# EloDoyard/movie-recommender-system

Measured on AMD Instinct MI355X. Metric: test-set predictions/sec (kNN k=300, fit+predict+MAE), higher is better.
Workload: dtype fp16 MFMA similarity filter (fp32 acc) + f64 exact re-rank/prediction

## Files before the change

### movie-recommender-system_amd/csrc/api.cpp

```cpp
#include <math.h>
#include <stdio.h>
#include <string.h>

#include <algorithm>
#include <vector>

#include "engine.h"

using namespace knncf;

namespace knncf {
void launch_first_rows(int64_t n, const int32_t* d_du, const int32_t* d_di, int32_t own_lo, int32_t own_hi,
                       uint32_t* d_first, hipStream_t st);
void launch_length_keys(int32_t count, const int32_t* d_list, const int64_t* d_u_ptr, int32_t max_len, uint64_t* d_key, hipStream_t st);
void launch_collect_new(int32_t U, const uint32_t* d_first, int64_t* d_seq, int64_t epoch, int32_t own_lo, int32_t own_hi,
                        int32_t* d_list, int32_t* d_count, hipStream_t st);
void launch_fallback_keys(int32_t U, const double* d_exact, uint64_t* d_keys, uint32_t* d_vals, hipStream_t st);
void launch_fallback_write(int32_t user, int32_t take, int32_t kcap, const uint32_t* d_sorted_vals,
                           const double* d_exact, int32_t* nbr_idx, double* nbr_sim, int32_t* nbr_cnt,
                           hipStream_t st);
void launch_jaccard_pair(const Train& tr, int32_t u, int32_t v, double* d_out, hipStream_t st);
}

struct StageTimer {
    hipEvent_t a, b;
    double* acc;
};

struct knncf_handle {
    knncf_config cfg{};
    hipStream_t stream = nullptr;
    std::string err;
    Train tr;
    PrepScratch prep;
    bool fitted = false, committed = false;
    int8_t short_rows = -1;
    NeighborTable nt;
    int64_t epoch = 1;
    int64_t U_pad = 0, K_pad = 0;
    DArr<bf16_t> Bpanel;
    bool b_ready = false;
    int32_t head = 0;
    double tail_pairs_full = 0.0;
    DArr<int32_t> colmap;
    DArr<int32_t> te_cnt, te_item;
    DArr<float> te_x, row_tail_abs, row_head_sq;
    DArr<float> row_len;
    hipStream_t stream2 = nullptr;
    DArr<bf16_t> Apanel[2];
    DArr<float> S[2];
    DArr<float> S_full;
    DArr<uint32_t> sym_tiles;
    DArr<int32_t> redo_rows;
    int32_t sym_tiles_n = 0;
    hipEvent_t ev_produced[2] = {nullptr, nullptr}, ev_consumed[2] = {nullptr, nullptr}, ev_ready = nullptr;
    int32_t* pinned_cnt = nullptr;
    size_t pinned_cap = 0;
    SelectScratch sel;
    SliceScratch slices;
    NeighborTable pt;
    bool pt_ready = false;
    PersonalRows prow;
    bool prow_ready = false;
    DArr<int32_t> reco_users, reco_items, reco_out_items;
    DArr<double> reco_pred, reco_out_preds;
    DArr<uint8_t> reco_rated;
    QueryBatchScratch query_batch;
    RecoBatchScratch reco_batch;
    DArr<int32_t> build_list, build_count;
    DArr<uint32_t> first_row;
    DArr<int32_t> t_du, t_di, t_users, t_items;
    DArr<double> t_pred, t_err, t_ratings, t_partial, scalar_out;
    DArr<unsigned long long> scalar_u64;
    DArr<uint8_t> t_owned;
    DArr<int64_t> t_counts;
    DArr<int32_t> sweep_ks;
    std::vector<uint32_t> h_ukeys, h_ikeys;
    std::vector<int32_t> h_uid;
    knncf_timings tm{};
    std::vector<StageTimer> pending;
    std::vector<hipEvent_t> event_pool;
};

namespace {

hipEvent_t get_event(knncf_handle* h) {
    if (!h->event_pool.empty()) {
        hipEvent_t e = h->event_pool.back();
        h->event_pool.pop_back();
        return e;
    }
    hipEvent_t e;
    KN_HIP(hipEventCreate(&e));
    return e;
}

struct Stage {
    knncf_handle* h;
    StageTimer t;
    hipStream_t st;
    Stage(knncf_handle* h_, double* acc, hipStream_t st_ = nullptr) : h(h_), st(st_ ? st_ : h_->stream) {
        t.a = get_event(h);
        t.b = get_event(h);
        t.acc = acc;
        (void)hipEventRecord(t.a, st);
    }
    ~Stage() {
        (void)hipEventRecord(t.b, st);
        h->pending.push_back(t);
// ... 7 lines not shown
        float ms = 0.f;
        if (hipEventElapsedTime(&ms, t.a, t.b) == hipSuccess) *t.acc += ms;
        h->event_pool.push_back(t.a);
        h->event_pool.push_back(t.b);
    }
    h->pending.clear();
}

template <class F>
int guarded(knncf_handle* h, F&& f) {
    if (!h) return KNNCF_E_INVALID;
    struct DeviceGuard {
        int prev = -1;
        ~DeviceGuard() { if (prev >= 0) (void)hipSetDevice(prev); }
    } guard;
    try {
        int cur = -1;
        if (hipGetDevice(&cur) != hipSuccess) {
            (void)hipGetLastError();
            KN_HIP(hipSetDevice(h->cfg.device));
        } else if (cur != h->cfg.device) {
            guard.prev = cur;
            KN_HIP(hipSetDevice(h->cfg.device));
        }
        f();
        resolve_timers(h);
        return KNNCF_OK;
    } catch (const Error& e) {
        h->err = e.what();
        (void)hipStreamSynchronize(h->stream);
        (void)hipStreamSynchronize(h->stream2);
        (void)hipGetLastError();
        h->pending.clear();
        return e.status;
    } catch (const std::bad_alloc&) {
        h->err = "host allocation failed";
        return KNNCF_E_NOMEM;
    } catch (const std::exception& e) {
        h->err = e.what();
        return KNNCF_E_INVALID;
    }
}

void require_fitted(knncf_handle* h, bool committed = true) {
    KN_REQUIRE(h->fitted, KNNCF_E_STATE, "call knncf_fit first");
    if (committed) KN_REQUIRE(h->committed, KNNCF_E_STATE, "sharded handle: call knncf_shard_commit after the exchange");
}

void load_host_ids(knncf_handle* h) {
    if (!h->h_ukeys.empty() || h->tr.U == 0) return;
    Train& tr = h->tr;
    h->h_ukeys.resize(tr.U);
    h->h_ikeys.resize(tr.I);
    h->h_uid.resize(tr.U);
    KN_HIP(hipMemcpyAsync(h->h_ukeys.data(), tr.ukeys.p, tr.U * sizeof(uint32_t), hipMemcpyDeviceToHost, h->stream));
    KN_HIP(hipMemcpyAsync(h->h_ikeys.data(), tr.ikeys.p, tr.I * sizeof(uint32_t), hipMemcpyDeviceToHost, h->stream));
    KN_HIP(hipMemcpyAsync(h->h_uid.data(), tr.uid.p, tr.U * sizeof(int32_t), hipMemcpyDeviceToHost, h->stream));
    KN_HIP(hipStreamSynchronize(h->stream));
}

int32_t dense_user(knncf_handle* h, int32_t raw) {
    load_host_ids(h);
    return dense_lookup(h->h_ukeys.data(), h->tr.U, raw);
}
int32_t dense_item(knncf_handle* h, int32_t raw) {
    load_host_ids(h);
// ... 83 lines not shown
        }
        if (tr.jaccard && (h->cfg.flags & KNNCF_FLAG_F32_PANEL) == 0) H = std::min(H, 2048);
    }
    h->tail_pairs_full = tail_sq[H];
    return H;
}

void build_neighbors(knncf_handle* h, int32_t count) {
    Train& tr = h->tr;
    NeighborTable& nt = h->nt;
    if (count <= 0 || nt.kcap <= 0) return;
    KN_REQUIRE(h->cfg.similarity != KNNCF_SIM_ONE, KNNCF_E_UNSUPPORTED,
               "kNN neighbourhoods with similarityOne: every similarity is 1.0, the neighbourhood is the first k users in Set order — not built");
    hipStream_t st = h->stream;
    if (count > 256) {
        PrepScratch& sc = h->prep;
        sc.k64_a.ensure(count); sc.k64_b.ensure(count); sc.v32_b.ensure(count);
        launch_length_keys(count, h->build_list.p, tr.u_ptr.p, tr.I, sc.k64_a.p, st);
        sort_pairs_u64_u32(sc.sort, sc.k64_a.p, sc.k64_b.p, reinterpret_cast<const uint32_t*>(h->build_list.p), sc.v32_b.p, count, bits_for((uint64_t)tr.I), st);
        KN_HIP(hipMemcpyAsync(h->build_list.p, sc.v32_b.p, (size_t)count * sizeof(int32_t), hipMemcpyDeviceToDevice, st));
    }
    const bool fp16 = (h->cfg.flags & KNNCF_FLAG_BF16_FILTER) == 0;
    const bool s_fp16 = (h->cfg.flags & KNNCF_FLAG_F32_PANEL) == 0;
    h->U_pad = round_up(tr.U, 256);
    const int64_t U_pad = h->U_pad;
    size_t free_b = 0, total_b = 0;
    KN_HIP(hipMemGetInfo(&free_b, &total_b));
    const int64_t s_elem = s_fp16 ? 2 : 4;
    const size_t sym_bytes = (size_t)U_pad * (size_t)U_pad * (size_t)s_elem;
    size_t own = h->S_full.bytes() + h->sel.cand_idx.bytes() + h->sel.cand_approx.bytes() + h->sel.grp_v0.bytes() + h->sel.grp_x.bytes();
    for (int s = 0; s < 2; ++s) own += h->S[s].bytes() + h->Apanel[s].bytes();
    bool use_sym = h->cfg.shard_count == 1 && (int64_t)count * 2 >= tr.U && U_pad / 256 < 65536 &&
                   sym_bytes <= (free_b + own) / 3 && !getenv("KNNCF_DEBUG_NO_SYMMETRIC_GEMM");
    if (use_sym) {
        try {
            h->S_full.ensure((sym_bytes + 3) / 4);
        } catch (const Error& e) {
            if (e.status != KNNCF_E_NOMEM) throw;
            (void)hipGetLastError();
            use_sym = false;
        }
    }
    if (!h->b_ready) {
        h->head = choose_head(h, count, use_sym);
        h->K_pad = round_up(h->head, 64);
        size_t need = (size_t)U_pad * h->K_pad * sizeof(bf16_t);
        KN_REQUIRE(need < free_b + h->Bpanel.bytes(), KNNCF_E_UNSUPPORTED,
                   "dense bf16 user panel does not fit in HBM; lower head_items");
        Stage s(h, &h->tm.densify_ms);
        h->colmap.ensure(tr.I);
        launch_colmap(tr, h->head, h->colmap.p, st);
        h->Bpanel.ensure((size_t)U_pad * h->K_pad);
        launch_densify(tr, nullptr, 0, tr.U, h->colmap.p, h->Bpanel.p, h->K_pad, U_pad, fp16, st);
        if (tr.jaccard) {
            KN_REQUIRE(!s_fp16 || h->head <= 2048, KNNCF_E_UNSUPPORTED, "Jaccard: more than 2048 dense head items need KNNCF_FLAG_F32_PANEL");
            h->row_len.ensure((size_t)row_len_size(tr.U));
            launch_row_len(tr, h->row_len.p, st);
        }
        if (h->head < tr.I) {
            h->te_cnt.ensure(tr.U); h->te_item.ensure(tr.n); h->te_x.ensure(tr.n);
            h->row_tail_abs.ensure(tr.U); h->row_head_sq.ensure(tr.U);
            launch_tail_entries(tr, h->colmap.p, h->te_cnt.p, h->te_item.p, h->te_x.p, h->row_tail_abs.p, h->row_head_sq.p, st);
        }
        h->b_ready = true;
        KN_HIP(hipMemGetInfo(&free_b, &total_b));
    }
    const int64_t K_pad = h->K_pad;
    const int32_t head = h->head;
    h->tm.head_items = head;
    if (use_sym) {
        const int32_t n_tiles = (int32_t)(U_pad / 256);
        if (h->sym_tiles_n != n_tiles) {
            std::vector<uint32_t> list;
            gemm_sym_tile_list(n_tiles, list);
            h->sym_tiles.ensure(list.size());
            KN_HIP(hipMemcpyAsync(h->sym_tiles.p, list.data(), list.size() * sizeof(uint32_t), hipMemcpyHostToDevice, st));
            KN_HIP(hipStreamSynchronize(st));
            h->sym_tiles_n = n_tiles;
        }
        const int64_t n_listed = (int64_t)n_tiles * (n_tiles + 1) / 2;
        Stage s(h, &h->tm.gemm_ms);
        launch_gemm_sym(h->Bpanel.p, h->S_full.p, s_fp16, U_pad, h->K_pad, h->K_pad, U_pad, fp16, !tr.jaccard, h->sym_tiles.p, n_listed, st);
        h->tm.gemm_launches += 1;
        h->tm.gemm_flops_executed += 2.0 * 256.0 * 256.0 * (double)n_listed * (double)h->K_pad;
        h->tm.gemm_flops_algorithmic += 2.0 * (double)count * (double)(tr.U - 1) * (double)h->head;
        KN_HIP(hipMemGetInfo(&free_b, &total_b));
    } else {
        h->S_full.release();
    }
    size_t held = 0;
    for (int s = 0; s < 2; ++s) held += h->S[s].bytes() + h->Apanel[s].bytes();
    held += h->sel.cand_idx.bytes() + h->sel.cand_approx.bytes() + h->sel.grp_v0.bytes() + h->sel.grp_x.bytes();
    int64_t budget = h->cfg.workspace_bytes > 0 ? h->cfg.workspace_bytes / 2
                                                : (int64_t)std::min<size_t>((size_t)48 << 30, (free_b + held) / 4);
    int64_t per_row = (use_sym ? 0 : U_pad * s_elem + K_pad * 2) + (int64_t)shortlist_cap(nt.k, tr.U) * 8 + (int64_t)select_gcap(nt.k) * 36;
    if (h->cfg.workspace_bytes <= 0) {
        const int64_t whole = round_up(count, 256) * per_row;
        if (whole <= (int64_t)std::min<size_t>((size_t)96 << 30, (free_b + held) / 3)) budget = std::max(budget, whole);
    }
    int64_t R = std::max<int64_t>(256, (budget / per_row) / 256 * 256);
    R = std::min<int64_t>(R, round_up(count, 256));
    const int64_t n_blocks = ceil_div(count, R);
    R = round_up(ceil_div(count, n_blocks), 256);
    const bool overlap = (h->cfg.flags & KNNCF_FLAG_OVERLAP) != 0;
    const int slots = (overlap && n_blocks > 1 && !use_sym) ? 2 : 1;
    for (int s = 0; s < slots && !use_sym; ++s) {
        h->S[s].ensure((size_t)(R * U_pad * s_elem + 3) / 4);
        h->Apanel[s].ensure((size_t)R * K_pad);
    }
    const int32_t cap = shortlist_cap(nt.k, tr.U);
    const bool verify = (h->cfg.flags & KNNCF_FLAG_VERIFY_BOUND) != 0;
    h->sel.cand_idx.ensure((size_t)R * cap);
    h->sel.cand_approx.ensure((size_t)R * cap);
    h->sel.cand_cnt.ensure(R);
    h->sel.cand_eps.ensure(R);
    h->sel.row_entries.ensure(R);
    h->sel.grp_v0.ensure((size_t)R * select_gcap(nt.k));
    h->sel.grp_x.ensure((size_t)R * select_gcap(nt.k) * 8);
    h->sel.stats.ensure(4);
    KN_HIP(hipMemsetAsync(h->sel.stats.p, 0, 4 * sizeof(double), st));
    if (h->pinned_cap < (size_t)count) {
        if (h->pinned_cnt) KN_HIP(hipHostFree(h->pinned_cnt));
        h->pinned_cnt = nullptr;
        h->pinned_cap = 0;
        KN_HIP(hipHostMalloc((void**)&h->pinned_cnt, (size_t)count * sizeof(int32_t), hipHostMallocDefault));
        h->pinned_cap = (size_t)count;
    }
    const float eps_opnd = gemm_eps_operand(fp16);
    const float eps_rest = gemm_eps_rest(fp16) + (s_fp16 ? 2.45e-4f : 0.f);
    hipStream_t sp = slots > 1 ? h->stream2 : h->stream;
    hipStream_t sc = h->stream;
    KN_HIP(hipEventRecord(h->ev_ready, sc));
    KN_HIP(hipStreamWaitEvent(sp, h->ev_ready, 0));
    std::vector<int32_t> h_rows;
    auto need_h_rows = [&] {
        if (!h_rows.empty()) return;
        h_rows.resize(count);
        KN_HIP(hipMemcpyAsync(h_rows.data(), h->build_list.p, (size_t)count * sizeof(int32_t), hipMemcpyDeviceToHost, st));
        KN_HIP(hipStreamSynchronize(st));
    };
    auto redo_marked = [&](const std::vector<int32_t>& marked, const void* Sp, bool by_user, int64_t rb) {
        need_h_rows();
        std::vector<int32_t> users(marked.size()), srow(marked.size());
        for (size_t j = 0; j < marked.size(); ++j) {
            users[j] = h_rows[marked[j]];
            srow[j] = (int32_t)(marked[j] - rb);
        }
        TailEntries te{h->te_cnt.p, h->te_item.p, h->te_x.p, h->row_tail_abs.p, h->row_head_sq.p, h->row_len.p};
        const int64_t chunk = std::min<int64_t>((int64_t)marked.size(), R);
        h->redo_rows.ensure(2 * (size_t)chunk);
        for (size_t j0 = 0; j0 < marked.size(); j0 += (size_t)R) {
            const int32_t m = (int32_t)std::min<size_t>((size_t)R, marked.size() - j0);
            KN_HIP(hipMemcpyAsync(h->redo_rows.p, users.data() + j0, (size_t)m * sizeof(int32_t), hipMemcpyHostToDevice, st));
            KN_HIP(hipMemcpyAsync(h->redo_rows.p + chunk, srow.data() + j0, (size_t)m * sizeof(int32_t), hipMemcpyHostToDevice, st));
            {
                Stage s(h, &h->tm.select_ms);
                launch_tail_select(tr, h->colmap.p, te, head < tr.I, Sp, by_user, s_fp16, U_pad, m, h->redo_rows.p, nt.k, eps_opnd, eps_rest, cap,
                                   h->sel.cand_idx.p, h->sel.cand_approx.p, h->sel.cand_cnt.p, h->sel.cand_eps.p, h->sel.grp_v0.p, h->sel.grp_x.p,
                                   select_gcap(nt.k), st, false, by_user ? nullptr : h->redo_rows.p + chunk);
                h->tm.select_launches += 1;
            }
            {
                Stage s(h, &h->tm.rerank_ms);
                launch_rerank(tr, nt, m, h->redo_rows.p, cap, h->sel.cand_idx.p, h->sel.cand_approx.p, h->sel.cand_cnt.p, h->sel.cand_eps.p,
                              h->sel.stats.p, h->sel.row_entries.p, verify, st);
            }
            std::vector<int32_t> again(m);
            KN_HIP(hipMemcpyAsync(again.data(), h->sel.cand_cnt.p, (size_t)m * sizeof(int32_t), hipMemcpyDeviceToHost, st));
            KN_HIP(hipStreamSynchronize(st));
            for (int32_t j = 0; j < m; ++j) h->pinned_cnt[marked[j0 + j]] = again[j];
        }
    };
    const bool per_block_redo = !use_sym && n_blocks > 1;
    for (int64_t b = 0; b < n_blocks; ++b) {
        const int64_t rb = b * R;
        const int32_t rows = (int32_t)std::min<int64_t>(R, count - rb);
        const int64_t M = round_up(rows, 256);
        const int32_t* d_rows = h->build_list.p + rb;
        const int slot = (int)(b % slots);
        if (b >= slots) KN_HIP(hipStreamWaitEvent(sp, h->ev_consumed[slot], 0));
        if (!use_sym) {
            Stage s(h, &h->tm.densify_ms, sp);
            launch_densify(tr, d_rows, 0, rows, h->colmap.p, h->Apanel[slot].p, K_pad, M, fp16, sp);
        }
        if (!use_sym) {
            Stage s(h, &h->tm.gemm_ms, sp);
            launch_gemm_nt(h->Apanel[slot].p, h->Bpanel.p, h->S[slot].p, s_fp16, M, U_pad, K_pad, K_pad, K_pad, U_pad, fp16, !tr.jaccard, sp);
            h->tm.gemm_launches += 1;
            h->tm.gemm_flops_executed += 2.0 * (double)M * (double)U_pad * (double)K_pad;
            h->tm.gemm_flops_algorithmic += 2.0 * (double)rows * (double)(tr.U - 1) * (double)head;
        }
        KN_HIP(hipEventRecord(h->ev_produced[slot], sp));
        KN_HIP(hipStreamWaitEvent(sc, h->ev_produced[slot], 0));
        TailEntries te{h->te_cnt.p, h->te_item.p, h->te_x.p, h->row_tail_abs.p, h->row_head_sq.p, h->row_len.p};
        h->prep.join_commit(sc);
        const void* Sblk = use_sym ? (const void*)h->S_full.p : (const void*)h->S[slot].p;
        const int32_t gcap = select_gcap(nt.k);
        auto select_rows = [&](int32_t r0, int32_t nr) {
            Stage s(h, &h->tm.select_ms, sc);
            const void* Sp = use_sym ? Sblk : (const void*)(static_cast<const char*>(Sblk) + (size_t)r0 * (size_t)U_pad * (size_t)s_elem);
            launch_tail_select(tr, h->colmap.p, te, head < tr.I, Sp, use_sym, s_fp16, U_pad, nr, d_rows + r0, nt.k, eps_opnd, eps_rest, cap,
                               h->sel.cand_idx.p + (size_t)r0 * cap, h->sel.cand_approx.p + (size_t)r0 * cap, h->sel.cand_cnt.p + r0, h->sel.cand_eps.p + r0,
                               h->sel.grp_v0.p + (size_t)r0 * gcap, h->sel.grp_x.p + (size_t)r0 * gcap * 8, gcap, sc);
            h->tm.select_launches += 1;
            h->tm.tail_pair_updates += h->tail_pairs_full * ((double)nr / (double)tr.U);
            h->tm.select_row_bytes += (double)s_elem * (double)nr * (double)tr.U;
        };
        const int32_t slices = std::min<int32_t>(8, 8192 / std::max<int32_t>(nt.kcap, 1));
        const char* force_slices = getenv("KNNCF_DEBUG_SLICE_ROWS");
        const int32_t n_heavy = slices < 2                         ? 0
                                : force_slices                     ? std::max<int32_t>(0, std::min<int32_t>(rows, atoi(force_slices)))
                                : (rows >= 4096 && rows <= 65536)  ? std::max<int32_t>(16, rows / 512)
                                                                   : 0;
        select_rows(0, rows);
        if (overlap && !per_block_redo) KN_HIP(hipEventRecord(h->ev_consumed[slot], sc));
        {
            Stage s(h, &h->tm.rerank_ms, sc);
            launch_rerank(tr, nt, rows, d_rows, cap, h->sel.cand_idx.p, h->sel.cand_approx.p, h->sel.cand_cnt.p, h->sel.cand_eps.p, h->sel.stats.p,
                          h->sel.row_entries.p, verify, sc, n_heavy, slices, &h->slices);
        }
        if (!overlap) KN_HIP(hipEventRecord(h->ev_consumed[slot], sc));
        if (per_block_redo) KN_HIP(hipMemcpyAsync(h->pinned_cnt + rb, h->sel.cand_cnt.p, rows * sizeof(int32_t), hipMemcpyDeviceToHost, sc));
        if (per_block_redo) {
            KN_HIP(hipStreamSynchronize(sc));
            std::vector<int32_t> marked;
            for (int64_t r = rb; r < rb + rows; ++r)
                if (h->pinned_cnt[r] > cap) marked.push_back((int32_t)r);
            if ((int64_t)marked.size() > std::max<int64_t>(64, rows / 200)) {
                redo_marked(marked, h->S[slot].p, false, rb);
            }
            if (overlap) KN_HIP(hipEventRecord(h->ev_consumed[slot], sc));
        }
    }
    const bool summary = !per_block_redo;
    unsigned long long four[4] = {0, 0, 0, 0};
    nt.by_id_valid = false;
    if (summary) KN_HIP(hipMemcpyAsync(four, h->sel.stats.p, sizeof(four), hipMemcpyDeviceToHost, sc));
    KN_HIP(hipStreamSynchronize(sc));
    KN_HIP(hipStreamSynchronize(sp));
    auto take_stats = [&](const unsigned long long* w) {
        h->tm.rerank_row_bytes += 12.0 * (double)w[1];
        if (verify && w[0] != 0) {
            double shifted;
            memcpy(&shifted, &w[0], sizeof(double));
            h->tm.max_bound_violation = std::max(h->tm.max_bound_violation, shifted - 4.0);
        }
// ... 15 lines not shown
    }
    for (int64_t r = 0; r < count; ++r) {
        h->tm.shortlist_total += std::min(h->pinned_cnt[r], cap);
        if (h->pinned_cnt[r] > cap) {
            need_h_rows();
            Stage s(h, &h->tm.rerank_ms);
            int32_t u = h_rows[r];
            h->sel.row_exact.ensure(tr.U);
            h->sel.fb_keys_a.ensure(tr.U); h->sel.fb_keys_b.ensure(tr.U);
            h->sel.fb_vals_a.ensure(tr.U); h->sel.fb_vals_b.ensure(tr.U);
            int64_t seq_u = fetch(h, nt.seq.p, u);
            launch_exact_row(tr, nt, u, seq_u, h->sel.row_exact.p, st);
            launch_fallback_keys(tr.U, h->sel.row_exact.p, h->sel.fb_keys_a.p, h->sel.fb_vals_a.p, st);
            sort_pairs_u64_u32(h->prep.sort, h->sel.fb_keys_a.p, h->sel.fb_keys_b.p, h->sel.fb_vals_a.p,
                               h->sel.fb_vals_b.p, tr.U, 64, st);
            launch_fallback_write(u, nt.kcap, nt.kcap, h->sel.fb_vals_b.p, h->sel.row_exact.p, nt.idx.p, nt.sim.p,
                                  nt.cnt.p, st);
            h->tm.fallback_rows += 1;
        }
    }
    {
        unsigned long long two[2] = {0, 0};
        KN_HIP(hipMemcpyAsync(two, h->sel.stats.p, sizeof(two), hipMemcpyDeviceToHost, st));
        KN_HIP(hipStreamSynchronize(st));
        take_stats(two);
    }
}

void ensure_test_scratch(knncf_handle* h, int64_t n) {
    h->t_du.ensure(n); h->t_di.ensure(n); h->t_pred.ensure(n); h->t_err.ensure(n); h->t_owned.ensure(n);
    h->t_partial.ensure(1024); h->t_counts.ensure(1024);
}

void ensure_neighbors_for_rows(knncf_handle* h, int64_t n) {
    Train& tr = h->tr;
    if (tr.U < 2 || h->nt.kcap <= 0) return;
    KN_REQUIRE(n < (int64_t)0xffffffffll, KNNCF_E_UNSUPPORTED, "more than 2^32-1 test rows");
    hipStream_t st = h->stream;
    h->first_row.ensure(tr.U);
    h->build_list.ensure(tr.U);
    h->build_count.ensure(1);
    KN_HIP(hipMemsetAsync(h->first_row.p, 0xff, tr.U * sizeof(uint32_t), st));
    KN_HIP(hipMemsetAsync(h->build_count.p, 0, sizeof(int32_t), st));
    launch_first_rows(n, h->t_du.p, h->t_di.p, 0, tr.U, h->first_row.p, st);
    launch_collect_new(tr.U, h->first_row.p, h->nt.seq.p, h->epoch, tr.own_lo, tr.own_hi, h->build_list.p, h->build_count.p, st);
    h->epoch += 1;
    int32_t count = fetch(h, h->build_count.p, 0);
    build_neighbors(h, count);
}

bool personalized_streams(const knncf_handle* h) { return h->tr.U > 2048 || getenv("KNNCF_DEBUG_PERSONALIZED_STREAM"); }

void require_personalized(knncf_handle* h) {
    Train& tr = h->tr;
    KN_REQUIRE(h->cfg.shard_count == 1, KNNCF_E_UNSUPPORTED, "PERSONALIZED is not sharded");
    if (h->cfg.similarity == KNNCF_SIM_COSINE) {
        std::vector<int64_t> ptr((size_t)tr.U + 1);
        KN_HIP(hipMemcpyAsync(ptr.data(), tr.u_ptr.p, ptr.size() * sizeof(int64_t), hipMemcpyDeviceToHost, h->stream));
        KN_HIP(hipStreamSynchronize(h->stream));
        for (int32_t u = 0; u < tr.U; ++u)
            KN_REQUIRE(ptr[u + 1] - ptr[u] > 4, KNNCF_E_UNSUPPORTED,
                       "PERSONALIZED with the adjusted cosine: a user with <= 4 ratings makes the reference's summation order depend on its memo history pair by pair (SURVEY N6); not modelled");
    }
}

void ensure_personalized_table(knncf_handle* h) {
    if (h->pt_ready) return;
    Train& tr = h->tr;
    require_personalized(h);
    NeighborTable& pt = h->pt;
    pt.k = pt.kcap = tr.U;
    const size_t cells = (size_t)tr.U * (size_t)tr.U;
    pt.uidx.ensure(cells);
    pt.usim.ensure(cells);
    pt.cnt.ensure(tr.U);
    launch_full_rows(tr, h->cfg.similarity == KNNCF_SIM_JACCARD, pt.uidx.p, pt.usim.p, pt.cnt.p, h->stream);
    pt.by_id_valid = true;
    h->pt_ready = true;
}

void ensure_personal_rows(knncf_handle* h) {
// ... 40 lines not shown
                                                          : (int64_t)std::min<size_t>((size_t)48 << 30, (free_b + pr.S.bytes()) / 4);
        R = std::min<int64_t>(std::max<int64_t>(1, budget / row_bytes), nu);
        R = ceil_div(nu, ceil_div(nu, R));
        pr.S.ensure((size_t)R * tr.U);
        std::vector<int32_t> slot((size_t)tr.U, -1);
        for (int64_t k = 0; k < nu; ++k) slot[users[k]] = (int32_t)(k % R);
        pr.users.ensure(nu);
        pr.slot.ensure(tr.U);
        KN_HIP(hipMemcpyAsync(pr.users.p, users.data(), (size_t)nu * sizeof(int32_t), hipMemcpyHostToDevice, st));
        KN_HIP(hipMemcpyAsync(pr.slot.p, slot.data(), (size_t)tr.U * sizeof(int32_t), hipMemcpyHostToDevice, st));
        KN_HIP(hipStreamSynchronize(st));
    }
    const int64_t n_blocks = std::max<int64_t>(1, ceil_div(nu, R));
    for (int64_t b = 0; b < n_blocks; ++b) {
        const int64_t u0 = b * R, u1 = std::min<int64_t>(nu, u0 + R);
        const int64_t r0 = b == 0 ? 0 : first_row[u0], r1 = b + 1 < n_blocks ? first_row[u1] : n;
        if (u1 > u0) {
            Stage s(h, &h->tm.rerank_ms);
            launch_sim_rows(tr, pr, pr.users.p + u0, (int32_t)(u1 - u0), pr.S.p, st);
        }
        Stage s(h, &h->tm.predict_ms);
        launch_fold_rows(tr, pr, r1 - r0, sc.v32_b.p + r0, h->t_du.p, h->t_di.p, d_ratings, pr.slot.p, pr.S.p, d_pred, h->t_err.p,
                         h->t_owned.p, st);
    }
}

void ensure_item_stats(knncf_handle* h) {
    if (h->tr.item_stats_ready) return;
    Stage s(h, &h->tm.prep_ms);
    h->prep.join_commit(h->stream);
    prep_item_stats(h->tr, h->prep, h->stream);
}

int64_t order_test_rows(knncf_handle* h, int64_t n, bool by_item, int32_t cols) {
    Train& tr = h->tr;
    hipStream_t st = h->stream;
    PrepScratch& sc = h->prep;
    sc.k64_a.ensure(n); sc.k64_b.ensure(n); sc.v32_a.ensure(n); sc.v32_b.ensure(n);
    const uint32_t key_limit = (uint32_t)(by_item ? tr.I : tr.U);
    if (h->cfg.shard_count > 1) {
        h->scalar_u64.ensure(1);
        KN_HIP(hipMemsetAsync(h->scalar_u64.p, 0, sizeof(unsigned long long), st));
        KN_HIP(hipMemsetAsync(h->t_err.p, 0, (size_t)cols * (size_t)n * sizeof(double), st));
        KN_HIP(hipMemsetAsync(h->t_owned.p, 0, (size_t)n, st));
        launch_owned_keys(n, by_item ? h->t_di.p : h->t_du.p, h->t_du.p, tr.own_lo, tr.own_hi, h->cfg.shard_rank == 0, key_limit,
                          sc.k64_a.p, sc.v32_a.p, h->scalar_u64.p, st);
        sort_pairs_u64_u32(sc.sort, sc.k64_a.p, sc.k64_b.p, sc.v32_a.p, sc.v32_b.p, n, bits_for((uint64_t)key_limit + 1), st);
        return (int64_t)fetch(h, h->scalar_u64.p, 0);
    }
    launch_user_keys(n, by_item ? h->t_di.p : h->t_du.p, key_limit, sc.k64_a.p, sc.v32_a.p, st);
    sort_pairs_u64_u32(sc.sort, sc.k64_a.p, sc.k64_b.p, sc.v32_a.p, sc.v32_b.p, n, bits_for((uint64_t)key_limit), st);
    return n;
}

void reduce_errors(knncf_handle* h, int64_t n, int32_t cols, double* sums, int64_t* count) {
    hipStream_t st = h->stream;
    const int32_t nb = 1024;
    h->t_partial.ensure((size_t)nb * cols);
    h->t_counts.ensure((size_t)nb * cols);
    for (int32_t c = 0; c < cols; ++c)
        launch_reduce_err(h->t_err.p + (size_t)c * n, h->t_owned.p, n, h->t_partial.p + (size_t)c * nb, h->t_counts.p + (size_t)c * nb, nb, st);
    std::vector<double> hp((size_t)nb * cols);
    std::vector<int64_t> hc((size_t)nb * cols);
    KN_HIP(hipMemcpyAsync(hp.data(), h->t_partial.p, hp.size() * sizeof(double), hipMemcpyDeviceToHost, st));
    KN_HIP(hipMemcpyAsync(hc.data(), h->t_counts.p, hc.size() * sizeof(int64_t), hipMemcpyDeviceToHost, st));
    KN_HIP(hipStreamSynchronize(st));
    for (int32_t c = 0; c < cols; ++c) {
        double s_ = 0.0;
        int64_t c_ = 0;
        for (int32_t b = 0; b < nb; ++b) { s_ += hp[(size_t)c * nb + b]; c_ += hc[(size_t)c * nb + b]; }
        if (sums) sums[c] = s_;
        if (count && c == 0) *count = c_;
    }
}

void run_predict(knncf_handle* h, int predictor, const int32_t* d_users, const int32_t* d_items,
                 const double* d_ratings, int64_t n, double* sum_abs_err, int64_t* count, double* d_pred_out) {
    require_fitted(h);
    Train& tr = h->tr;
    hipStream_t st = h->stream;
    KN_REQUIRE(n >= 0, KNNCF_E_INVALID, "negative row count");
    if (sum_abs_err) *sum_abs_err = 0.0;
    if (count) *count = 0;
    if (n == 0) return;
    KN_REQUIRE(d_users && d_items, KNNCF_E_INVALID, "null test arrays");
    int kind = predictor;
    NeighborTable* table = &h->nt;
    bool stream = false;
    if (predictor == KNNCF_PRED_PERSONALIZED) {
        if (h->cfg.similarity == KNNCF_SIM_ONE) {
            kind = KNNCF_PRED_BASELINE_RDD;
        } else if (personalized_streams(h)) {
            ensure_personal_rows(h);
            stream = true;
        } else {
            ensure_personalized_table(h);
            kind = KNNCF_PRED_KNN;
            table = &h->pt;
        }
    }
    KN_REQUIRE(stream || (kind >= KNNCF_PRED_GLOBAL_AVG && kind <= KNNCF_PRED_KNN), KNNCF_E_INVALID, "unknown predictor");
    if (kind == KNNCF_PRED_ITEM_AVG || kind == KNNCF_PRED_BASELINE || kind == KNNCF_PRED_BASELINE_RDD) ensure_item_stats(h);
    ensure_test_scratch(h, n);
    {
        Stage s(h, &h->tm.predict_ms);
        launch_dense_ids(tr, d_users, d_items, n, h->t_du.p, h->t_di.p, st);
    }
    if (kind == KNNCF_PRED_KNN && table == &h->nt) ensure_neighbors_for_rows(h, n);
    h->prep.join_commit(st);
    double* pred = d_pred_out ? d_pred_out : h->t_pred.p;
    if (stream) predict_personal_rows(h, d_ratings, n, pred);
    {
        Stage s(h, &h->tm.predict_ms);
        const uint32_t* d_order = nullptr;
        const bool by_item = tr.ib_words > 0 && lds_bitmap_fits(tr.ib_words);
        int64_t n_rows = n;
        if (kind == KNNCF_PRED_KNN) {
            n_rows = order_test_rows(h, n, by_item, 1);
            d_order = h->prep.v32_b.p;
        }
        if (n_rows > 0 && !stream)
            launch_predict(tr, table, kind, n_rows, h->t_du.p, h->t_di.p, d_ratings, d_order, by_item, pred, h->t_err.p, h->t_owned.p,
                           h->cfg.shard_rank == 0, st);
        if (sum_abs_err || count) reduce_errors(h, n, 1, sum_abs_err, count);
    }
}

void check_sweep_ks(const int32_t* ks, int32_t n_k) {
    KN_REQUIRE(ks && n_k >= 1 && n_k <= 64, KNNCF_E_INVALID, "sweep: 1 .. 64 values of k");
    for (int32_t q = 0; q < n_k; ++q)
        KN_REQUIRE(ks[q] >= 1 && ks[q] <= 2048 && (q == 0 || ks[q] > ks[q - 1]), KNNCF_E_INVALID,
                   "sweep: k must be strictly ascending in [1, 2048]");
}

void run_mae_sweep(knncf_handle* h, const int32_t* ks, int32_t n_k, const int32_t* d_users, const int32_t* d_items,
                   const double* d_ratings, int64_t n, double* sums, int64_t* count, double* d_pred) {
    check_sweep_ks(ks, n_k);
    require_fitted(h);
    KN_REQUIRE(h->cfg.similarity != KNNCF_SIM_ONE, KNNCF_E_UNSUPPORTED,
               "kNN neighbourhoods with similarityOne: every similarity is 1.0, the neighbourhood is the first k users in Set order — not built");
    KN_REQUIRE(n >= 0, KNNCF_E_INVALID, "negative row count");
    for (int32_t q = 0; q < n_k; ++q) sums[q] = 0.0;
    *count = 0;
    if (n == 0) return;
    KN_REQUIRE(d_users && d_items && d_ratings, KNNCF_E_INVALID, "null test arrays");
    Train& tr = h->tr;
    hipStream_t st = h->stream;
    struct Restore {
        knncf_handle* h;
        int32_t k;
        ~Restore() {
            h->cfg.k = k;
            try { reset_neighbors(h); } catch (const Error&) {}
        }
    } restore{h, h->cfg.k};
    h->cfg.k = ks[n_k - 1];
    reset_neighbors(h);
    ensure_test_scratch(h, n);
    h->t_err.ensure((size_t)n_k * n);
    {
        Stage s(h, &h->tm.predict_ms);
        launch_dense_ids(tr, d_users, d_items, n, h->t_du.p, h->t_di.p, st);
    }
    ensure_neighbors_for_rows(h, n);
    h->prep.join_commit(st);
    std::vector<int32_t> hk(ks, ks + n_k);
    h->sweep_ks.ensure(64);
    KN_HIP(hipMemcpyAsync(h->sweep_ks.p, hk.data(), (size_t)n_k * sizeof(int32_t), hipMemcpyHostToDevice, st));
    {
        Stage s(h, &h->tm.predict_ms);
        const int64_t n_rows = order_test_rows(h, n, true, n_k);
        if (n_rows > 0)
            launch_predict_sweep(tr, h->nt, h->sweep_ks.p, n_k, n_rows, n, h->t_du.p, h->t_di.p, d_ratings, h->prep.v32_b.p, d_pred,
                                 h->t_err.p, h->t_owned.p, h->cfg.shard_rank == 0, st);
        reduce_errors(h, n, n_k, sums, count);
    }
}

void do_fit_device(knncf_handle* h, const int32_t* d_users, const int32_t* d_items, const double* d_ratings, int64_t n) {
    KN_REQUIRE(n > 0 && d_users && d_items && d_ratings, KNNCF_E_INVALID, "fit: null or empty input");
    Train& tr = h->tr;
    hipStream_t st = h->stream;
    h->fitted = h->committed = false;
    h->short_rows = -1;
    h->b_ready = false;
    h->pt_ready = false;
    h->prow_ready = false;
    h->h_ukeys.clear(); h->h_ikeys.clear(); h->h_uid.clear();
    tr.n = n;
    tr.jaccard = h->cfg.similarity == KNNCF_SIM_JACCARD;
    {
        Stage s(h, &h->tm.prep_ms);
        if (tr.user_raw.p != d_users) {
            tr.user_raw.alloc(n); tr.item_raw.alloc(n); tr.rating.alloc(n);
            KN_HIP(hipMemcpyAsync(tr.user_raw.p, d_users, n * sizeof(int32_t), hipMemcpyDeviceToDevice, st));
            KN_HIP(hipMemcpyAsync(tr.item_raw.p, d_items, n * sizeof(int32_t), hipMemcpyDeviceToDevice, st));
            KN_HIP(hipMemcpyAsync(tr.rating.p, d_ratings, n * sizeof(double), hipMemcpyDeviceToDevice, st));
        }
        prep_fit(tr, h->prep, h->cfg.shard_rank, h->cfg.shard_count, st);
    }
    h->fitted = true;
    reset_neighbors(h);
    if (h->cfg.shard_count == 1) {
        Stage s(h, &h->tm.prep_ms);
        prep_commit(tr, h->prep, st);
        h->committed = true;
// ... 345 lines not shown
        case KNNCF_E_DUPLICATE: return "duplicate (user,item) rating";
        case KNNCF_E_NOMEM: return "out of memory";
        case KNNCF_E_HIP: return "HIP runtime error";
        case KNNCF_E_STATE: return "invalid call order";
        case KNNCF_E_UNSUPPORTED: return "unsupported configuration";
        case KNNCF_E_NODEVICE: return "no usable gfx950 device";
        case KNNCF_E_RCCL: return "RCCL error";
        default: return "unknown status";
    }
}

int knncf_create(const knncf_config* cfg, knncf_handle** out) {
    if (!cfg || !out || cfg->struct_size != sizeof(knncf_config)) return KNNCF_E_INVALID;
    if (cfg->shard_count < 1 || cfg->shard_rank < 0 || cfg->shard_rank >= cfg->shard_count || cfg->k < 0)
        return KNNCF_E_INVALID;
    if (cfg->similarity < KNNCF_SIM_COSINE || cfg->similarity > KNNCF_SIM_JACCARD) return KNNCF_E_INVALID;
    int ndev = 0;
    if (hipGetDeviceCount(&ndev) != hipSuccess || ndev <= 0 || cfg->device < 0 || cfg->device >= ndev) {
        (void)hipGetLastError();
        return KNNCF_E_NODEVICE;
    }
    hipDeviceProp_t prop;
    if (hipGetDeviceProperties(&prop, cfg->device) != hipSuccess) return KNNCF_E_NODEVICE;
    if (strncmp(prop.gcnArchName, "gfx950", 6) != 0) return KNNCF_E_NODEVICE;
    knncf_handle* h = new (std::nothrow) knncf_handle();
    if (!h) return KNNCF_E_NOMEM;
    h->cfg = *cfg;
    if (hipSetDevice(cfg->device) != hipSuccess || hipStreamCreateWithFlags(&h->stream, hipStreamNonBlocking) != hipSuccess ||
        hipStreamCreateWithFlags(&h->stream2, hipStreamNonBlocking) != hipSuccess) {
        delete h;
        return KNNCF_E_HIP;
    }
    bool ok = hipEventCreateWithFlags(&h->ev_ready, hipEventDisableTiming) == hipSuccess;
    for (int s = 0; s < 2; ++s) {
        ok = ok && hipEventCreateWithFlags(&h->ev_produced[s], hipEventDisableTiming) == hipSuccess;
        ok = ok && hipEventCreateWithFlags(&h->ev_consumed[s], hipEventDisableTiming) == hipSuccess;
    }
    if (!ok) {
        knncf_destroy(h);
        return KNNCF_E_HIP;
    }
    *out = h;
    return KNNCF_OK;
}

void knncf_destroy(knncf_handle* h) {
    if (!h) return;
    (void)hipSetDevice(h->cfg.device);
    (void)hipStreamSynchronize(h->stream);
    for (auto& t : h->pending) { (void)hipEventDestroy(t.a); (void)hipEventDestroy(t.b); }
    for (auto e : h->event_pool) (void)hipEventDestroy(e);
    if (h->stream2) (void)hipStreamSynchronize(h->stream2);
    if (h->ev_ready) (void)hipEventDestroy(h->ev_ready);
    for (int s = 0; s < 2; ++s) {
        if (h->ev_produced[s]) (void)hipEventDestroy(h->ev_produced[s]);
        if (h->ev_consumed[s]) (void)hipEventDestroy(h->ev_consumed[s]);
    }
    if (h->pinned_cnt) (void)hipHostFree(h->pinned_cnt);
    if (h->stream2) (void)hipStreamDestroy(h->stream2);
    (void)hipStreamDestroy(h->stream);
    delete h;
}

const char* knncf_last_error(const knncf_handle* h) { return h ? h->err.c_str() : "null handle"; }

int knncf_fit_device(knncf_handle* h, const int32_t* d_users, const int32_t* d_items, const double* d_ratings, int64_t n) {
    return guarded(h, [&] { do_fit_device(h, d_users, d_items, d_ratings, n); });
}

int knncf_fit(knncf_handle* h, const int32_t* users, const int32_t* items, const double* ratings, int64_t n) {
    return guarded(h, [&] {
        KN_REQUIRE(n > 0 && users && items && ratings, KNNCF_E_INVALID, "fit: null or empty input");
        Train& tr = h->tr;
        tr.user_raw.alloc(n); tr.item_raw.alloc(n); tr.rating.alloc(n);
        KN_HIP(hipMemcpyAsync(tr.user_raw.p, users, n * sizeof(int32_t), hipMemcpyHostToDevice, h->stream));
        KN_HIP(hipMemcpyAsync(tr.item_raw.p, items, n * sizeof(int32_t), hipMemcpyHostToDevice, h->stream));
        KN_HIP(hipMemcpyAsync(tr.rating.p, ratings, n * sizeof(double), hipMemcpyHostToDevice, h->stream));
        do_fit_device(h, tr.user_raw.p, tr.item_raw.p, tr.rating.p, n);
    });
}

int knncf_num_users(const knncf_handle* h, int32_t* out) {
    if (!h || !out || !h->fitted) return KNNCF_E_STATE;
    *out = h->tr.U;
    return KNNCF_OK;
}
// ... 535 lines not shown
```

Before: 85.76 million.

## Overlap tail-list build and test-row ordering with neighbor build on side stream

Tail-entry and row-length construction now run on the second stream after colmap, concurrently with densify and GEMM, and are joined only where the redo and select steps need them. Test-row key sorting moves to dedicated buffers and can run on the side stream beside the neighbor build. The post-build hipMemGetInfo calls are dropped in favour of bookkeeping over buffer sizes, and the symmetric tile list is uploaded earlier. This hides small kernels and host syncs behind the main build, at the cost of more events, extra scratch memory and cross-stream ordering that must stay correct.

After: 85.59 million. About the same (-0.2%).

```diff
diff --git a/movie-recommender-system_amd/csrc/api.cpp b/movie-recommender-system_amd/csrc/api.cpp
--- a/movie-recommender-system_amd/csrc/api.cpp
+++ b/movie-recommender-system_amd/csrc/api.cpp
@@ -54,6 +54,9 @@
     DArr<int32_t> redo_rows;
     int32_t sym_tiles_n = 0;
     hipEvent_t ev_produced[2] = {nullptr, nullptr}, ev_consumed[2] = {nullptr, nullptr}, ev_ready = nullptr;
+    hipEvent_t ev_colmap = nullptr, ev_tail = nullptr, ev_rows = nullptr;
+    bool tail_pending = false, rows_pending = false;
+    struct { bool want = false; int64_t n = 0; bool by_item = false; int32_t cols = 0; } rows_deferred;
     int32_t* pinned_cnt = nullptr;
     size_t pinned_cap = 0;
     SelectScratch sel;
@@ -75,6 +78,9 @@
     DArr<uint8_t> t_owned;
     DArr<int64_t> t_counts;
     DArr<int32_t> sweep_ks;
+    SortWorkspace t_sort;
+    DArr<uint64_t> t_k64_a, t_k64_b;
+    DArr<uint32_t> t_v32_a, t_order;
     std::vector<uint32_t> h_ukeys, h_ikeys;
     std::vector<int32_t> h_uid;
     knncf_timings tm{};
@@ -148,6 +154,7 @@
         (void)hipStreamSynchronize(h->stream2);
         (void)hipGetLastError();
         h->pending.clear();
+        h->tail_pending = h->rows_pending = h->rows_deferred.want = false;
         return e.status;
     } catch (const std::bad_alloc&) {
         h->err = "host allocation failed";
@@ -297,6 +304,7 @@
     for (int s = 0; s < 2; ++s) own += h->S[s].bytes() + h->Apanel[s].bytes();
     bool use_sym = h->cfg.shard_count == 1 && (int64_t)count * 2 >= tr.U && U_pad / 256 < 65536 &&
                    sym_bytes <= (free_b + own) / 3 && !getenv("KNNCF_DEBUG_NO_SYMMETRIC_GEMM");
+    const size_t s_full_before = h->S_full.bytes();
     if (use_sym) {
         try {
             h->S_full.ensure((sym_bytes + 3) / 4);
@@ -306,53 +314,86 @@
             use_sym = false;
         }
     }
+    auto build_bytes = [&] {
+        return h->S_full.bytes() + h->Bpanel.bytes() + h->colmap.bytes() + h->te_cnt.bytes() + h->te_item.bytes() + h->te_x.bytes() +
+               h->row_tail_abs.bytes() + h->row_head_sq.bytes() + h->row_len.bytes() + h->sym_tiles.bytes();
+    };
+    const size_t bytes_at_query = build_bytes() - h->S_full.bytes() + s_full_before;
+    const int32_t n_tiles = (int32_t)(U_pad / 256);
+    if (use_sym && h->sym_tiles_n != n_tiles) {
+        std::vector<uint32_t> list;
+        gemm_sym_tile_list(n_tiles, list);
+        h->sym_tiles.ensure(list.size());
+        KN_HIP(hipMemcpyAsync(h->sym_tiles.p, list.data(), list.size() * sizeof(uint32_t), hipMemcpyHostToDevice, st));
+        KN_HIP(hipStreamSynchronize(st));
+        h->sym_tiles_n = n_tiles;
+    }
+    const bool overlap = (h->cfg.flags & KNNCF_FLAG_OVERLAP) != 0;
+    auto launch_tail_lists = [&](hipStream_t side) {
+        {
+            Stage s(h, &h->tm.densify_ms, side);
+            if (tr.jaccard) launch_row_len(tr, h->row_len.p, side);
+            if (h->head < tr.I)
+                launch_tail_entries(tr, h->colmap.p, h->te_cnt.p, h->te_item.p, h->te_x.p, h->row_tail_abs.p, h->row_head_sq.p, side);
+        }
+        if (side != h->stream) {
+            KN_HIP(hipEventRecord(h->ev_tail, side));
+            h->tail_pending = true;
+        }
+    };
+    auto join_tail_lists = [&](hipStream_t consumer) {
+        if (!h->tail_pending) return;
+        KN_HIP(hipStreamWaitEvent(consumer, h->ev_tail, 0));
+        h->tail_pending = false;
+    };
+    bool tail_deferred = false;
     if (!h->b_ready) {
         h->head = choose_head(h, count, use_sym);
         h->K_pad = round_up(h->head, 64);
         size_t need = (size_t)U_pad * h->K_pad * sizeof(bf16_t);
         KN_REQUIRE(need < free_b + h->Bpanel.bytes(), KNNCF_E_UNSUPPORTED,
                    "dense bf16 user panel does not fit in HBM; lower head_items");
-        Stage s(h, &h->tm.densify_ms);
+        KN_REQUIRE(!tr.jaccard || !s_fp16 || h->head <= 2048, KNNCF_E_UNSUPPORTED, "Jaccard: more than 2048 dense head items need KNNCF_FLAG_F32_PANEL");
+        const bool has_tail = h->head < tr.I;
         h->colmap.ensure(tr.I);
-        launch_colmap(tr, h->head, h->colmap.p, st);
         h->Bpanel.ensure((size_t)U_pad * h->K_pad);
-        launch_densify(tr, nullptr, 0, tr.U, h->colmap.p, h->Bpanel.p, h->K_pad, U_pad, fp16, st);
-        if (tr.jaccard) {
-            KN_REQUIRE(!s_fp16 || h->head <= 2048, KNNCF_E_UNSUPPORTED, "Jaccard: more than 2048 dense head items need KNNCF_FLAG_F32_PANEL");
-            h->row_len.ensure((size_t)row_len_size(tr.U));
-            launch_row_len(tr, h->row_len.p, st);
-        }
-        if (h->head < tr.I) {
+        if (tr.jaccard) h->row_len.ensure((size_t)row_len_size(tr.U));
+        if (has_tail) {
             h->te_cnt.ensure(tr.U); h->te_item.ensure(tr.n); h->te_x.ensure(tr.n);
             h->row_tail_abs.ensure(tr.U); h->row_head_sq.ensure(tr.U);
-            launch_tail_entries(tr, h->colmap.p, h->te_cnt.p, h->te_item.p, h->te_x.p, h->row_tail_abs.p, h->row_head_sq.p, st);
+        }
+        {
+            Stage s(h, &h->tm.densify_ms);
+            launch_colmap(tr, h->head, h->colmap.p, st);
+            KN_HIP(hipEventRecord(h->ev_colmap, st));
+            launch_densify(tr, nullptr, 0, tr.U, h->colmap.p, h->Bpanel.p, h->K_pad, U_pad, fp16, st);
+        }
+        if (tr.jaccard || has_tail) {
+            if (overlap && !use_sym) {
+                tail_deferred = true;
+            } else {
+                KN_HIP(hipStreamWaitEvent(h->stream2, h->ev_colmap, 0));
+                launch_tail_lists(h->stream2);
+            }
         }
         h->b_ready = true;
-        KN_HIP(hipMemGetInfo(&free_b, &total_b));
     }
     const int64_t K_pad = h->K_pad;
     const int32_t head = h->head;
     h->tm.head_items = head;
     if (use_sym) {
-        const int32_t n_tiles = (int32_t)(U_pad / 256);
-        if (h->sym_tiles_n != n_tiles) {
-            std::vector<uint32_t> list;
-            gemm_sym_tile_list(n_tiles, list);
-            h->sym_tiles.ensure(list.size());
-            KN_HIP(hipMemcpyAsync(h->sym_tiles.p, list.data(), list.size() * sizeof(uint32_t), hipMemcpyHostToDevice, st));
-            KN_HIP(hipStreamSynchronize(st));
-            h->sym_tiles_n = n_tiles;
-        }
         const int64_t n_listed = (int64_t)n_tiles * (n_tiles + 1) / 2;
         Stage s(h, &h->tm.gemm_ms);
         launch_gemm_sym(h->Bpanel.p, h->S_full.p, s_fp16, U_pad, h->K_pad, h->K_pad, U_pad, fp16, !tr.jaccard, h->sym_tiles.p, n_listed, st);
         h->tm.gemm_launches += 1;
         h->tm.gemm_flops_executed += 2.0 * 256.0 * 256.0 * (double)n_listed * (double)h->K_pad;
         h->tm.gemm_flops_algorithmic += 2.0 * (double)count * (double)(tr.U - 1) * (double)h->head;
-        KN_HIP(hipMemGetInfo(&free_b, &total_b));
-    } else {
-        h->S_full.release();
-    }
+    }
+    {
+        const size_t now = build_bytes();
+        free_b = now >= bytes_at_query ? free_b - std::min(free_b, now - bytes_at_query) : free_b + (bytes_at_query - now);
+    }
+    if (!use_sym) h->S_full.release();
     size_t held = 0;
     for (int s = 0; s < 2; ++s) held += h->S[s].bytes() + h->Apanel[s].bytes();
     held += h->sel.cand_idx.bytes() + h->sel.cand_approx.bytes() + h->sel.grp_v0.bytes() + h->sel.grp_x.bytes();
@@ -367,7 +408,6 @@
     R = std::min<int64_t>(R, round_up(count, 256));
     const int64_t n_blocks = ceil_div(count, R);
     R = round_up(ceil_div(count, n_blocks), 256);
-    const bool overlap = (h->cfg.flags & KNNCF_FLAG_OVERLAP) != 0;
     const int slots = (overlap && n_blocks > 1 && !use_sym) ? 2 : 1;
     for (int s = 0; s < slots && !use_sym; ++s) {
         h->S[s].ensure((size_t)(R * U_pad * s_elem + 3) / 4);
@@ -397,6 +437,11 @@
     hipStream_t sc = h->stream;
     KN_HIP(hipEventRecord(h->ev_ready, sc));
     KN_HIP(hipStreamWaitEvent(sp, h->ev_ready, 0));
+    if (tail_deferred) {
+        hipStream_t side = slots > 1 ? sc : h->stream2;
+        if (side != sc) KN_HIP(hipStreamWaitEvent(side, h->ev_ready, 0));
+        launch_tail_lists(side);
+    }
     std::vector<int32_t> h_rows;
     auto need_h_rows = [&] {
         if (!h_rows.empty()) return;
@@ -412,6 +457,7 @@
             srow[j] = (int32_t)(marked[j] - rb);
         }
         TailEntries te{h->te_cnt.p, h->te_item.p, h->te_x.p, h->row_tail_abs.p, h->row_head_sq.p, h->row_len.p};
+        join_tail_lists(st);
         const int64_t chunk = std::min<int64_t>((int64_t)marked.size(), R);
         h->redo_rows.ensure(2 * (size_t)chunk);
         for (size_t j0 = 0; j0 < marked.size(); j0 += (size_t)R) {
@@ -477,6 +523,7 @@
                                 : force_slices                     ? std::max<int32_t>(0, std::min<int32_t>(rows, atoi(force_slices)))
                                 : (rows >= 4096 && rows <= 65536)  ? std::max<int32_t>(16, rows / 512)
                                                                    : 0;
+        join_tail_lists(sc);
         select_rows(0, rows);
         if (overlap && !per_block_redo) KN_HIP(hipEventRecord(h->ev_consumed[slot], sc));
         {
@@ -558,9 +605,9 @@
     h->t_partial.ensure(1024); h->t_counts.ensure(1024);
 }
 
-void ensure_neighbors_for_rows(knncf_handle* h, int64_t n) {
+int32_t collect_neighbors_for_rows(knncf_handle* h, int64_t n) {
     Train& tr = h->tr;
-    if (tr.U < 2 || h->nt.kcap <= 0) return;
+    if (tr.U < 2 || h->nt.kcap <= 0) return 0;
     KN_REQUIRE(n < (int64_t)0xffffffffll, KNNCF_E_UNSUPPORTED, "more than 2^32-1 test rows");
     hipStream_t st = h->stream;
     h->first_row.ensure(tr.U);
@@ -571,8 +618,7 @@
     launch_first_rows(n, h->t_du.p, h->t_di.p, 0, tr.U, h->first_row.p, st);
     launch_collect_new(tr.U, h->first_row.p, h->nt.seq.p, h->epoch, tr.own_lo, tr.own_hi, h->build_list.p, h->build_count.p, st);
     h->epoch += 1;
-    int32_t count = fetch(h, h->build_count.p, 0);
-    build_neighbors(h, count);
+    return fetch(h, h->build_count.p, 0);
 }
 
 bool personalized_streams(const knncf_handle* h) { return h->tr.U > 2048 || getenv("KNNCF_DEBUG_PERSONALIZED_STREAM"); }
@@ -679,25 +725,59 @@
     prep_item_stats(h->tr, h->prep, h->stream);
 }
 
-int64_t order_test_rows(knncf_handle* h, int64_t n, bool by_item, int32_t cols) {
+void order_test_rows(knncf_handle* h, int64_t n, bool by_item, int32_t cols, hipStream_t st) {
     Train& tr = h->tr;
-    hipStream_t st = h->stream;
-    PrepScratch& sc = h->prep;
-    sc.k64_a.ensure(n); sc.k64_b.ensure(n); sc.v32_a.ensure(n); sc.v32_b.ensure(n);
     const uint32_t key_limit = (uint32_t)(by_item ? tr.I : tr.U);
     if (h->cfg.shard_count > 1) {
-        h->scalar_u64.ensure(1);
         KN_HIP(hipMemsetAsync(h->scalar_u64.p, 0, sizeof(unsigned long long), st));
         KN_HIP(hipMemsetAsync(h->t_err.p, 0, (size_t)cols * (size_t)n * sizeof(double), st));
         KN_HIP(hipMemsetAsync(h->t_owned.p, 0, (size_t)n, st));
         launch_owned_keys(n, by_item ? h->t_di.p : h->t_du.p, h->t_du.p, tr.own_lo, tr.own_hi, h->cfg.shard_rank == 0, key_limit,
-                          sc.k64_a.p, sc.v32_a.p, h->scalar_u64.p, st);
-        sort_pairs_u64_u32(sc.sort, sc.k64_a.p, sc.k64_b.p, sc.v32_a.p, sc.v32_b.p, n, bits_for((uint64_t)key_limit + 1), st);
-        return (int64_t)fetch(h, h->scalar_u64.p, 0);
-    }
-    launch_user_keys(n, by_item ? h->t_di.p : h->t_du.p, key_limit, sc.k64_a.p, sc.v32_a.p, st);
-    sort_pairs_u64_u32(sc.sort, sc.k64_a.p, sc.k64_b.p, sc.v32_a.p, sc.v32_b.p, n, bits_for((uint64_t)key_limit), st);
-    return n;
+                          h->t_k64_a.p, h->t_v32_a.p, h->scalar_u64.p, st);
+        sort_pairs_u64_u32(h->t_sort, h->t_k64_a.p, h->t_k64_b.p, h->t_v32_a.p, h->t_order.p, n, bits_for((uint64_t)key_limit + 1), st);
+        return;
+    }
+    launch_user_keys(n, by_item ? h->t_di.p : h->t_du.p, key_limit, h->t_k64_a.p, h->t_v32_a.p, st);
+    sort_pairs_u64_u32(h->t_sort, h->t_k64_a.p, h->t_k64_b.p, h->t_v32_a.p, h->t_order.p, n, bits_for((uint64_t)key_limit), st);
+}
+int64_t ordered_row_count(knncf_handle* h, int64_t n) {
+    return h->cfg.shard_count > 1 ? (int64_t)fetch(h, h->scalar_u64.p, 0) : n;
+}
+
+void fork_test_order(knncf_handle* h);
+void queue_test_order(knncf_handle* h, int64_t n, bool by_item, int32_t cols, bool beside_build) {
+    h->t_k64_a.ensure(n); h->t_k64_b.ensure(n); h->t_v32_a.ensure(n); h->t_order.ensure(n);
+    if (h->cfg.shard_count > 1) h->scalar_u64.ensure(1);
+    if (beside_build && (h->cfg.flags & KNNCF_FLAG_OVERLAP) == 0) {
+        h->rows_deferred.want = true;
+        h->rows_deferred.n = n; h->rows_deferred.by_item = by_item; h->rows_deferred.cols = cols;
+        fork_test_order(h);
+        return;
+    }
+    Stage s(h, &h->tm.predict_ms);
+    order_test_rows(h, n, by_item, cols, h->stream);
+}
+void fork_test_order(knncf_handle* h) {
+    if (!h->rows_deferred.want) return;
+    h->rows_deferred.want = false;
+    KN_HIP(hipEventRecord(h->ev_rows, h->stream));
+    KN_HIP(hipStreamWaitEvent(h->stream2, h->ev_rows, 0));
+    {
+        Stage s(h, &h->tm.predict_ms, h->stream2);
+        order_test_rows(h, h->rows_deferred.n, h->rows_deferred.by_item, h->rows_deferred.cols, h->stream2);
+    }
+    KN_HIP(hipEventRecord(h->ev_rows, h->stream2));
+    h->rows_pending = true;
+}
+void join_test_order(knncf_handle* h) {
+    if (h->rows_deferred.want) {
+        h->rows_deferred.want = false;
+        Stage s(h, &h->tm.predict_ms);
+        order_test_rows(h, h->rows_deferred.n, h->rows_deferred.by_item, h->rows_deferred.cols, h->stream);
+    }
+    if (!h->rows_pending) return;
+    KN_HIP(hipStreamWaitEvent(h->stream, h->ev_rows, 0));
+    h->rows_pending = false;
 }
 
 void reduce_errors(knncf_handle* h, int64_t n, int32_t cols, double* sums, int64_t* count) {
@@ -753,18 +833,23 @@
         Stage s(h, &h->tm.predict_ms);
         launch_dense_ids(tr, d_users, d_items, n, h->t_du.p, h->t_di.p, st);
     }
-    if (kind == KNNCF_PRED_KNN && table == &h->nt) ensure_neighbors_for_rows(h, n);
+    const bool by_item = tr.ib_words > 0 && lds_bitmap_fits(tr.ib_words);
+    if (kind == KNNCF_PRED_KNN) {
+        const int32_t count = table == &h->nt ? collect_neighbors_for_rows(h, n) : 0;
+        queue_test_order(h, n, by_item, 1, count > 0);
+        build_neighbors(h, count);
+    }
     h->prep.join_commit(st);
     double* pred = d_pred_out ? d_pred_out : h->t_pred.p;
     if (stream) predict_personal_rows(h, d_ratings, n, pred);
     {
         Stage s(h, &h->tm.predict_ms);
         const uint32_t* d_order = nullptr;
-        const bool by_item = tr.ib_words > 0 && lds_bitmap_fits(tr.ib_words);
         int64_t n_rows = n;
         if (kind == KNNCF_PRED_KNN) {
-            n_rows = order_test_rows(h, n, by_item, 1);
-            d_order = h->prep.v32_b.p;
+            join_test_order(h);
+            n_rows = ordered_row_count(h, n);
+            d_order = h->t_order.p;
         }
         if (n_rows > 0 && !stream)
             launch_predict(tr, table, kind, n_rows, h->t_du.p, h->t_di.p, d_ratings, d_order, by_item, pred, h->t_err.p, h->t_owned.p,
@@ -809,16 +894,21 @@
         Stage s(h, &h->tm.predict_ms);
         launch_dense_ids(tr, d_users, d_items, n, h->t_du.p, h->t_di.p, st);
     }
-    ensure_neighbors_for_rows(h, n);
+    {
+        const int32_t count = collect_neighbors_for_rows(h, n);
+        queue_test_order(h, n, true, n_k, count > 0);
+        build_neighbors(h, count);
+    }
     h->prep.join_commit(st);
     std::vector<int32_t> hk(ks, ks + n_k);
     h->sweep_ks.ensure(64);
     KN_HIP(hipMemcpyAsync(h->sweep_ks.p, hk.data(), (size_t)n_k * sizeof(int32_t), hipMemcpyHostToDevice, st));
     {
         Stage s(h, &h->tm.predict_ms);
-        const int64_t n_rows = order_test_rows(h, n, true, n_k);
+        join_test_order(h);
+        const int64_t n_rows = ordered_row_count(h, n);
         if (n_rows > 0)
-            launch_predict_sweep(tr, h->nt, h->sweep_ks.p, n_k, n_rows, n, h->t_du.p, h->t_di.p, d_ratings, h->prep.v32_b.p, d_pred,
+            launch_predict_sweep(tr, h->nt, h->sweep_ks.p, n_k, n_rows, n, h->t_du.p, h->t_di.p, d_ratings, h->t_order.p, d_pred,
                                  h->t_err.p, h->t_owned.p, h->cfg.shard_rank == 0, st);
         reduce_errors(h, n, n_k, sums, count);
     }
@@ -1230,6 +1320,7 @@
         return KNNCF_E_HIP;
     }
     bool ok = hipEventCreateWithFlags(&h->ev_ready, hipEventDisableTiming) == hipSuccess;
+    for (hipEvent_t* e : {&h->ev_colmap, &h->ev_tail, &h->ev_rows}) ok = ok && hipEventCreateWithFlags(e, hipEventDisableTiming) == hipSuccess;
     for (int s = 0; s < 2; ++s) {
         ok = ok && hipEventCreateWithFlags(&h->ev_produced[s], hipEventDisableTiming) == hipSuccess;
         ok = ok && hipEventCreateWithFlags(&h->ev_consumed[s], hipEventDisableTiming) == hipSuccess;
@@ -1250,6 +1341,8 @@
     for (auto e : h->event_pool) (void)hipEventDestroy(e);
     if (h->stream2) (void)hipStreamSynchronize(h->stream2);
     if (h->ev_ready) (void)hipEventDestroy(h->ev_ready);
+    for (hipEvent_t e : {h->ev_colmap, h->ev_tail, h->ev_rows})
+        if (e) (void)hipEventDestroy(e);
     for (int s = 0; s < 2; ++s) {
         if (h->ev_produced[s]) (void)hipEventDestroy(h->ev_produced[s]);
         if (h->ev_consumed[s]) (void)hipEventDestroy(h->ev_consumed[s]);
```
